# seceq/zkir

Measured on AMD Instinct MI355X. Metric: trace rows/sec (2^20-cycle fib: execution-trace fill + BabyBear NTT/LDE + Poseidon2 Merkle commitment), higher is better.
Workload: dtype u32 (Baby Bear, 31-bit modular) / u64 trace words

## Files before the change

include/zkir_amd.h:

```cpp
#ifndef ZKIR_AMD_H
#define ZKIR_AMD_H

#include <stddef.h>
#include <stdint.h>

#ifdef __cplusplus
extern "C" {
#endif

enum {
  ZKIR_OK = 0,
  ZKIR_ERR_MISALIGNED = 1,
  ZKIR_ERR_INVALID_MEMORY = 2,
  ZKIR_ERR_DIV_ZERO = 3,
  ZKIR_ERR_INVALID_SYSCALL = 4,
  ZKIR_ERR_DECODE = 5,
  ZKIR_ERR_OTHER = 6,
  ZKIR_ERR_BAD_PROGRAM = 7,
  ZKIR_ERR_DEVICE = 8,
  ZKIR_ERR_ARGUMENT = 9
};

enum { ZKIR_HALT_EBREAK = 0, ZKIR_HALT_EXIT = 1, ZKIR_HALT_CYCLE_LIMIT = 2 };

// ... 170 lines not shown
void zkir_stark_ctx_free(zkir_stark_ctx* ctx);
uint32_t zkir_main_trace_width(void);
uint32_t zkir_main_trace_width_for(uint32_t deferred);
uint32_t zkir_padded_log_n(uint64_t n_real);
int zkir_main_trace_launch(const zkir_trace_columns* trace, uint64_t n_real, uint32_t deferred, uint32_t* out, void* hip_stream);
typedef struct zkir_io_args { const uint64_t* inputs; uint64_t n_inputs; uint64_t writes_before, reads_before; } zkir_io_args;
int zkir_main_trace_io_launch(const zkir_trace_columns* trace, uint64_t n_real, const zkir_io_args* io, uint32_t* scratch, uint32_t* out, void* hip_stream);
int zkir_main_trace_io_host(const zkir_trace_columns* trace, uint64_t n_real, const zkir_io_args* io, uint32_t* out);
int zkir_main_trace_mem_launch(const zkir_trace_columns* trace, uint64_t n_real, const zkir_io_args* io, const uint64_t* mem_old, const uint32_t* mem_told, uint32_t* scratch, uint32_t* out,
                               void* hip_stream);
int zkir_main_trace_mem_host(const zkir_trace_columns* trace, uint64_t n_real, const zkir_io_args* io, const uint64_t* mem_old, const uint32_t* mem_told, uint32_t* out);
int zkir_main_trace_wide_launch(const zkir_trace_columns* trace, uint64_t n_real, const zkir_io_args* io, const uint64_t* mem_old, const uint32_t* mem_told, uint64_t code_size,
                                uint32_t* scratch, uint32_t* out, void* hip_stream);
int zkir_main_trace_wide_host(const zkir_trace_columns* trace, uint64_t n_real, const zkir_io_args* io, const uint64_t* mem_old, const uint32_t* mem_told, uint64_t code_size, uint32_t* out);
int zkir_main_trace_host(const zkir_trace_columns* trace, uint64_t n_real, uint32_t deferred, uint32_t* out);
void zkir_air_eval_host(const uint32_t* loc, const uint32_t* nxt, const uint32_t* aloc, const uint32_t* anxt, const uint32_t* lk, uint32_t is_first, uint32_t is_last, uint32_t is_trans,
                        const uint32_t* first68, const uint32_t* last68, const uint32_t* alpha4, uint32_t mode ,
                        const uint32_t* cnt4 , uint32_t* out4);
int zkir_air_check_bounds(uint32_t deferred, char* why, size_t why_len);
int zkir_lde_launch(const zkir_stark_ctx* ctx, uint32_t* in, uint32_t width, uint32_t* out, void* hip_stream);
int zkir_merkle_commit_launch(const zkir_stark_ctx* ctx, const uint32_t* mat, uint32_t width, uint64_t n_leaves, uint32_t* tree, void* hip_stream);

int zkir_merkle_leaves_launch(const zkir_stark_ctx* ctx, const uint32_t* mat, uint32_t width, uint64_t n_leaves, uint32_t* digests, void* hip_stream);

int zkir_merkle_cap_launch(const zkir_stark_ctx* ctx, uint32_t* tree, uint64_t n_digests, void* hip_stream);

typedef struct zkir_public_inputs {
  uint64_t n_real;
  uint64_t entry_point;
  uint32_t deferred;
  uint32_t fri_params;
  uint32_t program_digest[4];
  uint32_t io_digest[4];
  const uint8_t* program_blob;
  uint64_t program_blob_len;
  const uint64_t* inputs;
  uint64_t n_inputs;
  const uint64_t* outputs;
  uint64_t n_outputs;
  uint32_t halt_kind;
  uint32_t reserved2;
  uint64_t halt_code;
  uint64_t writes_before, reads_before;
  const uint64_t* mem_old;
  const uint32_t* mem_told;
  const uint64_t* cell_addr;
// ... 44 lines not shown
  uint32_t num_queries;
  uint32_t pow_bits;
} zkir_prover_params;
int zkir_public_inputs_set_params(zkir_public_inputs* pub, const zkir_prover_params* params);

int zkir_prove(const zkir_stark_ctx* ctx, const zkir_trace_columns* trace, const zkir_public_inputs* pub, uint32_t** proof_out, uint64_t* proof_words,
               float* stage_ms, void* hip_stream);
void zkir_proof_free(uint32_t* proof);
int zkir_prove_result(const zkir_result* result, const zkir_prover_params* params, uint8_t** proof, size_t* proof_len);
void zkir_proof_bytes_free(uint8_t* proof);
uint32_t zkir_proof_num_queries(void);
uint32_t zkir_proof_version(void);
uint32_t zkir_proof_version_of_mode(uint32_t mode);
int zkir_verify(const uint32_t* proof, uint64_t proof_words, const zkir_public_inputs* expect);
int zkir_verify_segment(const uint32_t* proof, uint64_t proof_words, const zkir_public_inputs* expect, uint32_t first_state[68], uint32_t last_state[68]);
int zkir_verify_chain(const uint32_t* const* proofs, const uint64_t* proof_words, uint32_t n_segments, const zkir_public_inputs* expect);
int zkir_verify_io(const uint32_t* proof, uint64_t words, const zkir_public_inputs* expect, const uint64_t* inputs, size_t n_inputs, const uint64_t* outputs, size_t n_outputs,
                   int halt_kind, uint64_t halt_code);
int zkir_verify_chain_io(const uint32_t* const* proofs, const uint64_t* words, uint32_t n_segments, const zkir_public_inputs* expect, const uint64_t* inputs, size_t n_inputs,
                         const uint64_t* outputs, size_t n_outputs, int halt_kind, uint64_t halt_code);
uint32_t zkir_proof_state_words(void);
void zkir_poseidon2_permute(uint32_t state[12]);
void zkir_poseidon2_permute_scaled(uint32_t state[12], uint32_t rounds);


int zkir_exec(const uint8_t* program_blob, size_t blob_len, const uint64_t* inputs, size_t n_inputs,
              const zkir_vm_config* cfg, zkir_result** out);
int zkir_exec_window(const uint8_t* program_blob, size_t blob_len, const uint64_t* inputs, size_t n_inputs, const zkir_vm_config* cfg,
                     uint64_t row_begin, uint64_t row_end, zkir_result** out);
int zkir_exec_shard(const zkir_delta_log* log, uint64_t row_begin, uint64_t row_end, zkir_result** out);
void zkir_result_free(zkir_result* r);
const zkir_delta_log* zkir_result_delta_log(const zkir_result* r);
const zkir_trace_columns* zkir_result_trace(const zkir_result* r);
void zkir_result_stage_ms(const zkir_result* r, float out[4]);
int zkir_result_copy_column(const zkir_result* r, int field, int reg, void* dst);


typedef struct zkir_memory_witness {
  uint64_t n_ops;
  uint64_t n_rows;
  zkir_memop_columns row_order;
  const uint64_t* row_offsets;
  zkir_memop_columns sorted;
} zkir_memory_witness;
int zkir_result_memory_trace(zkir_result* r, zkir_memory_witness* out);

// ... 41 lines not shown
```

zkir_amd/csrc/babybear.h:

```cpp
#pragma once
#include <cstdint>

#if defined(__HIPCC__)
#define BB_HD __host__ __device__ __forceinline__
#else
#define BB_HD inline
#endif

namespace bb {

constexpr uint32_t P = 0x78000001u;
constexpr uint32_t NEG_PINV = 0x77FFFFFFu;
constexpr uint32_t R1 = 0x0FFFFFFEu;
constexpr uint32_t R2 = 0x45DDDDE3u;
constexpr uint32_t GEN = 31u;
constexpr uint32_t ROOT27 = 0x1A427A41u;
constexpr uint32_t W_EXT = 11u;

BB_HD uint32_t add(uint32_t a, uint32_t b) { const uint32_t s = a + b, d = s - P; return d < s ? d : s; }
BB_HD uint32_t sub(uint32_t a, uint32_t b) { const uint32_t d = a - b, e = d + P; return e < d ? e : d; }
BB_HD uint32_t neg(uint32_t a) { return a ? P - a : 0u; }
BB_HD uint32_t dbl(uint32_t a) { return add(a, a); }
BB_HD uint32_t mont_mul(uint32_t a, uint32_t b) {
  const uint64_t t = (uint64_t)a * b;
// ... 138 lines not shown
#endif
}
BB_HD int32_t wredc(int64_t acc) {
#if defined(__HIP_DEVICE_COMPILE__)
  const int32_t m = (int32_t)((uint32_t)acc * NEG_PINV);
  return (int32_t)((uint64_t)wmadk<(int32_t)P>(acc, m) >> 32);
#else
  return smont_reduce_wide(acc);
#endif
}
BB_HD int32_t centre(uint32_t w) { const uint32_t u = w + (uint32_t)W_HALF, d = u - P; return (int32_t)((d < u ? d : u) - (uint32_t)W_HALF); }
BB_HD uint32_t wcanon(int32_t x) { const uint32_t u = (uint32_t)x, s = u + P; return s < u ? s : u; }
BB_HD int32_t mont_mul_centred(uint32_t a, uint32_t b) {
#if defined(__HIP_DEVICE_COMPILE__)
  uint64_t t, u;
  asm("v_mad_u64_u32 %0, vcc, %1, %2, %3" : "=v"(t) : "v"(a), "v"(b), "s"((uint64_t)(uint32_t)W_HALF << 32) : "vcc");
  const uint32_t m = (uint32_t)t * NEG_PINV;
  asm("v_mad_u64_u32 %0, vcc, %1, %2, %3" : "=v"(u) : "v"(m), "s"(P), "v"(t) : "vcc");
  return (int32_t)(reduce_2p((uint32_t)(u >> 32)) - (uint32_t)W_HALF);
#else
  return (int32_t)(reduce_2p(mont_mul_add_lazy(a, b, (uint64_t)(uint32_t)W_HALF << 32)) - (uint32_t)W_HALF);
#endif
}
BB_HD void dit2w(int32_t& a, int32_t& b, int32_t w, int32_t nw) {
  const int64_t A = wmulk<W_ONE>(a);
  const int32_t b0 = b;
  a = wredc(wmad(A, b0, w)); b = wredc(wmad(A, b0, nw));
}
BB_HD void dit4w(int32_t& x0, int32_t& x1, int32_t& x2, int32_t& x3, int32_t w1, int32_t n1, int32_t w2, int32_t n2, int32_t w2i, int32_t n2i) {
  const int64_t X0 = wmulk<W_ONE>(x0), X2 = wmulk<W_ONE>(x2);
  const int64_t y0 = wmad(X0, x1, w1), y1 = wmad(X0, x1, n1);
  const int32_t y2 = wredc(wmad(X2, x3, w1)), y3 = wredc(wmad(X2, x3, n1));
  x0 = wredc(wmad(y0, y2, w2)); x2 = wredc(wmad(y0, y2, n2));
  x1 = wredc(wmad(y1, y3, w2i)); x3 = wredc(wmad(y1, y3, n2i));
}
BB_HD void dit4w2(int32_t* a, int32_t* b, int32_t w1, int32_t n1, int32_t w2, int32_t n2, int32_t w2i, int32_t n2i) {
#if defined(__HIP_DEVICE_COMPILE__)
  int64_t ay0, ay1, at2, at3, by0, by1, bt2, bt3;
  asm("v_mad_i64_i32 %1, vcc, %8, %18, 0\n\tv_mad_i64_i32 %5, vcc, %12, %18, 0\n\t"
      "v_mad_i64_i32 %3, vcc, %10, %18, 0\n\tv_mad_i64_i32 %7, vcc, %14, %18, 0\n\t"
      "v_mad_i64_i32 %0, vcc, %9, %16, %1\n\tv_mad_i64_i32 %4, vcc, %13, %16, %5\n\t"
      "v_mad_i64_i32 %2, vcc, %11, %16, %3\n\tv_mad_i64_i32 %6, vcc, %15, %16, %7\n\t"
      "v_mad_i64_i32 %1, vcc, %9, %17, %1\n\tv_mad_i64_i32 %5, vcc, %13, %17, %5\n\t"
      "v_mad_i64_i32 %3, vcc, %11, %17, %3\n\tv_mad_i64_i32 %7, vcc, %15, %17, %7"
      : "=&v"(ay0), "=&v"(ay1), "=&v"(at2), "=&v"(at3), "=&v"(by0), "=&v"(by1), "=&v"(bt2), "=&v"(bt3)
      : "v"(a[0]), "v"(a[1]), "v"(a[2]), "v"(a[3]), "v"(b[0]), "v"(b[1]), "v"(b[2]), "v"(b[3]), "v"(w1), "v"(n1), "s"(W_ONE) : "vcc");
// ... 117 lines not shown
```

zkir_amd/csrc/ntt.hip:

```cpp
#include <hip/hip_runtime.h>

#include <atomic>
#include <cstdlib>
#include <mutex>
#include <type_traits>

#include "../../include/zkir_amd.h"
#include "../../include/zkir_amd_experimental.h"
#include "babybear.h"
#include "host.h"

namespace {

constexpr int NT = 256;
__device__ __forceinline__ uint32_t bitrev(uint32_t x, int bits) { return bits == 0 ? 0u : __brev(x) >> (32 - bits); }

template <int K, int N, class F>
__device__ __forceinline__ void static_for(F&& f) {
  if constexpr (K < N) { f(std::integral_constant<int, K>{}); static_for<K + 1, N>(f); }
}

using u32x4 = uint32_t __attribute__((ext_vector_type(4)));
__device__ __forceinline__ u32x4 ld4(const uint4* p) { return *reinterpret_cast<const u32x4*>(p); }
__device__ __forceinline__ void st4(uint4* p, u32x4 v) { *reinterpret_cast<u32x4*>(p) = v; }
// ... 336 lines not shown
    uint32_t v[2];
    int cnt = 0;
    for (uint32_t e = threadIdx.x; e < n; e += NT) { const uint32_t k = bitrev(e, L); v[cnt++] = bb::mont_mul(bb::mont_mul(lds[e], g_lo[k & 1023]), g_hi[k >> 10]); }
    __syncthreads();
    cnt = 0;
    for (uint32_t e = threadIdx.x; e < n; e += NT) { lds[2 * e] = v[cnt]; lds[2 * e + 1] = v[cnt]; cnt++; }
    __syncthreads();
    for (int s = 1; s <= L; s++) {
      const uint32_t half = 1u << s;
      for (uint32_t q = threadIdx.x; q < n; q += NT) {
        const uint32_t r_lo = q & (half - 1), r_hi = q >> s;
        const uint32_t ia = (r_hi << (s + 1)) | r_lo, ib = ia + half;
        const uint32_t a = lds[ia], t = bb::mont_mul(lds[ib], small_fwd[r_lo << (L - s)]);
        lds[ia] = bb::add(a, t); lds[ib] = bb::sub(a, t);
      }
      __syncthreads();
    }
    for (uint32_t e = threadIdx.x; e < 2 * n; e += NT) y[(uint64_t)e * 8 + c] = lds[e];
    __syncthreads();
  }
}

constexpr int MID_NT = 512;
__global__ __launch_bounds__(MID_NT) __attribute__((amdgpu_waves_per_eu(4, 4))) void lde_middle_r4_kernel(const uint4* __restrict__ in, uint4* __restrict__ out, uint32_t chunks_per_block, uint32_t total, int L,
                                                                const uint32_t* __restrict__ tw_inv, const uint32_t* __restrict__ small_inv, const uint32_t* __restrict__ small_fwd,
                                                                const uint32_t* __restrict__ g_lo, const uint32_t* __restrict__ g_hi, uint32_t j4_inv_m, uint32_t j4_fwd_m, int canon) {
  constexpr int Bm = 10;
  constexpr uint32_t APL = 1024;
  __shared__ uint4 A[2 * APL];
  __shared__ uint4 Bf[2048];
  const uint32_t n = 1u << L, t = threadIdx.x;
  uint32_t w = blockIdx.x;
  if (w >= total) return;
  uint32_t tw_i[5], tw_f[5];
#pragma unroll
  for (int r = 0; r < 5; r++) {
    const int lg = 8 - 2 * r;
    tw_i[r] = small_inv[bitrev((t & 255) >> lg, 2 * r) << lg];
    const int sft = 2 * r + 1;
    tw_f[r] = small_fwd[(t & ((1u << sft) - 1)) << (Bm - sft - 1)];
  }
  u32x4 pre[4];
  uint32_t cf_next[5];
  uint32_t glo[4], ghi[4];
  auto fetch = [&](uint32_t ww) {
    const uint4* x = in + ((uint64_t)(ww / chunks_per_block) * n + ((uint64_t)(ww % chunks_per_block) << Bm)) * 2;
#pragma unroll
    for (int k = 0; k < 4; k++) pre[k] = ld4(&x[t + k * MID_NT]);
    const uint32_t p0 = ((ww % chunks_per_block) << Bm) + 4 * (t & 255);
#pragma unroll
    for (int i = 0; i < 4; i++) { const uint32_t k = bitrev(p0 + i, L); glo[i] = g_lo[k & 1023]; ghi[i] = g_hi[k >> 10]; }
    const uint32_t ce = bitrev(ww % chunks_per_block, L - Bm);
#pragma unroll
    for (int r = 0; r < 5; r++) cf_next[r] = tw_inv[ce << (8 - 2 * r)];
  };
  fetch(w);
  for (;;) {
    const uint32_t base = (w % chunks_per_block) << Bm;
    uint4* y = out + (uint64_t)(w / chunks_per_block) * n * 4;
#pragma unroll
    for (int k = 0; k < 4; k++) { const uint32_t e = t + k * MID_NT; st4(&A[(e & 1) * APL + (e >> 1)], pre[k]); }
    uint32_t gs[4];
#pragma unroll
    for (int i = 0; i < 4; i++) gs[i] = bb::mont_mul(glo[i], ghi[i]);
// ... 11 lines not shown
        const int lg = 8 - 2 * r;
        const uint32_t h2 = 1u << lg, lo = q & (h2 - 1), hi = q >> lg;
        const uint32_t i0 = (hi << (lg + 2)) | lo;
        WTw c1, c2, c2i;
        ct_twiddles(tw_i[r], cf[r], false, j4_inv_m, c1, c2, c2i);
        uint4 x0 = a[i0], x1 = a[i0 + h2], x2 = a[i0 + 2 * h2], x3 = a[i0 + 3 * h2];
        ct4w4(x0, x1, x2, x3, c1, c2, c2i);
        if (r == 4) {
          x0 = scale4(x0, gs[0]); x1 = scale4(x1, gs[1]); x2 = scale4(x2, gs[2]); x3 = scale4(x3, gs[3]);
        }
        a[i0] = x0; a[i0 + h2] = x1; a[i0 + 2 * h2] = x2; a[i0 + 3 * h2] = x3;
        if (r >= 1 && r < 4) wave_sync_lds(); else __syncthreads();
      }
    }
#pragma unroll 1
    for (int h = 0; h < 2; h++) {
      const uint4* a = A + h * APL;
      uint4* F = h == 0 ? Bf : A;
#pragma unroll
      for (int r = 0; r < 5; r++) {
        const int s = 2 * r + 1;
        const uint32_t lo = t & ((1u << s) - 1), hi = t >> s;
        const uint32_t i0 = (hi << (s + 2)) | lo, d = 1u << s;
        const uint32_t w2 = tw_f[r];
        const WTw c2 = wtw(bb::centre(w2)), c1 = wtw(bb::mont_mul_centred(w2, w2)), c2i = wtw(bb::mont_mul_centred(w2, j4_fwd_m));
        uint4 x0, x1, x2, x3;
        if (r == 0) {
          x0 = a[i0 >> 1]; x1 = a[(i0 + d) >> 1]; x2 = a[(i0 + 2 * d) >> 1]; x3 = a[(i0 + 3 * d) >> 1];
          __syncthreads();
        } else { x0 = F[i0]; x1 = F[i0 + d]; x2 = F[i0 + 2 * d]; x3 = F[i0 + 3 * d]; }
        dit4w4(x0, x1, x2, x3, c1, c2, c2i);
        F[i0] = x0; F[i0 + d] = x1; F[i0 + 2 * d] = x2; F[i0 + 3 * d] = x3;
        if (r < 2) wave_sync_lds(); else __syncthreads();
      }
    }
#pragma unroll
    for (int k = 0; k < 4; k++) {
      const uint32_t e = t + k * MID_NT;
      uint4 v0 = Bf[e], v1 = A[e];
      if (canon) { v0 = canon4(v0); v1 = canon4(v1); }
      y[((uint64_t)2 * base + e) * 2] = v0; y[((uint64_t)2 * base + e) * 2 + 1] = v1;
    }
    __syncthreads();
    if (wn >= total) break;
    w = wn;
  }
}

// ... 75 lines not shown
```

zkir_amd/csrc/poseidon2.h:

```cpp
#pragma once
#include "babybear.h"

#ifndef P2_RF_UNROLL
#define P2_RF_UNROLL 1
#endif
namespace p2 {

constexpr int T = 12, RF = 8, RP = 22, RATE = 8, DIGEST = 4;

struct Consts {
  uint32_t ext[RF][T];
  uint32_t in[RP];
  uint32_t diag[T];
  uint32_t pre[RF][T];
  uint32_t ext0_s[T];
  uint64_t pre_b[RF][T];
  uint32_t in_scale;
  uint32_t out_scale;
  uint32_t carry;
  int32_t in0_neg;
  int32_t pr_c[RP];
  uint64_t pr_a[RP];
  uint64_t pr_k[T];
};

inline uint64_t splitmix64(uint64_t& s) {
  uint64_t z = (s += 0x9E3779B97F4A7C15ull);
// ... 227 lines not shown
  }
  int_round_a(x, t, w, c, RP - 1);
  s[0] = (uint32_t)x;
#pragma unroll
  for (int i = 1; i < T; i++) s[i] = (uint32_t)bb::smont_reduce_wide((int64_t)((uint64_t)w[i] + c.pr_k[i]));
}
BB_HD void permute_scaled(uint32_t* s, const Consts& c) {
  ext_linear_scaled<true>(s, c.ext0_s);
#pragma unroll P2_RF_UNROLL
  for (int r = 0; r < RF / 2; r++) {
#pragma unroll
    for (int i = 0; i < T; i++) s[i] = sbox_biased(s[i], c.pre_b[r][i]);
    ext_linear_scaled<false>(s, nullptr);
  }
  int_rounds_scaled(s, c);
#pragma unroll P2_RF_UNROLL
  for (int r = RF / 2; r < RF; r++) {
#pragma unroll
    for (int i = 0; i < T; i++) s[i] = sbox_biased(s[i], c.pre_b[r][i]);
    ext_linear_scaled<false>(s, nullptr);
  }
}

#if defined(__HIPCC__)
template <int CTRL>
__device__ __forceinline__ uint32_t quad_perm(uint32_t v) { return (uint32_t)__builtin_amdgcn_mov_dpp((int)v, CTRL, 0xF, 0xF, true); }
template <int CTRL>
__device__ __forceinline__ uint64_t quad_perm64(uint64_t v) { return ((uint64_t)quad_perm<CTRL>((uint32_t)(v >> 32)) << 32) | quad_perm<CTRL>((uint32_t)v); }

template <bool ADD_RC>
__device__ __forceinline__ void ext_linear_quad_scaled(uint32_t* s, const uint32_t* m4row, const uint32_t* rc) {
  uint64_t y[3];
#pragma unroll
  for (int b = 0; b < 3; b++) {
    const uint32_t v0 = quad_perm<0x00>(s[b]), v1 = quad_perm<0x55>(s[b]), v2 = quad_perm<0xAA>(s[b]), v3 = quad_perm<0xFF>(s[b]);
    y[b] = (uint64_t)v0 * m4row[0] + (uint64_t)v1 * m4row[1] + (uint64_t)v2 * m4row[2] + (uint64_t)v3 * m4row[3];
  }
  const uint64_t sum = y[0] + y[1] + y[2];
#pragma unroll
  for (int b = 0; b < 3; b++) {
    uint64_t v = y[b] + sum;
    if (ADD_RC) v += rc[b];
    s[b] = bb::mont_reduce_wide(v);
  }
}
__device__ __forceinline__ void int_round_quad(int32_t& x, int64_t* w, uint64_t mask0, const int* k, const Consts& c, int r) {
// ... 106 lines not shown
```

zkir_amd/csrc/stark.hip:

```cpp
#include <hip/hip_runtime.h>

#include <array>
#include <atomic>
#include <chrono>
#include <cstdio>
#include <cstdlib>
#include <cstddef>
#include <memory>
#include <mutex>
#include <vector>

#include "../../include/zkir_amd.h"
#include "../../include/zkir_amd_experimental.h"
#include "air.h"
#include "babybear.h"
#include "host.h"
#include "hashcall.h"
#include "poseidon2.h"
#include "verify_stages.h"

namespace {

constexpr int NT = 256;

// ... 420 lines not shown
  uint32_t d[8], pre[8];
  uint32_t run = bb::R1;
#pragma unroll
  for (int k = 0; k < 8; k++) {
    const uint32_t j = j0 + k;
    const uint32_t wj = j < N ? tw_fwd[j] : bb::neg(tw_fwd[j - N]);
    d[k] = bb::sub(bb::mont_mul(wj, bb::to_mont(bb::GEN)), bb::R1);
    pre[k] = run; run = bb::mont_mul(run, d[k]);
  }
  uint32_t inv = bb::R1, b = run, e = bb::P - 2;
  while (e) { if (e & 1) inv = bb::mont_mul(inv, b); b = bb::mont_mul(b, b); e >>= 1; }
#pragma unroll
  for (int k = 7; k >= 0; k--) { inv_xm1[j0 + k] = bb::mont_mul(inv, pre[k]); inv = bb::mont_mul(inv, d[k]); }
}


__global__ __launch_bounds__(NT) void leaf_hash_kernel(const p2::Consts* __restrict__ cp, const uint32_t* __restrict__ mat, uint32_t width, uint64_t n, uint32_t in_scale, uint32_t* __restrict__ digests) {
  const uint64_t j = (uint64_t)blockIdx.x * NT + threadIdx.x;
  if (j >= n) return;
  uint32_t s[p2::T];
#pragma unroll
  for (int i = 0; i < p2::T; i++) s[i] = 0;
  const uint4* m4 = reinterpret_cast<const uint4*>(mat);
  const uint32_t carry = cp->carry, out_scale = cp->out_scale;
  for (uint32_t off = 0; off < width; off += p2::RATE) {
    const uint4 lo = m4[((uint64_t)(off >> 3) * n + j) * 2], hi = m4[((uint64_t)(off >> 3) * n + j) * 2 + 1];
    const uint32_t v[8] = {lo.x, lo.y, lo.z, lo.w, hi.x, hi.y, hi.z, hi.w};
#pragma unroll
    for (int i = 0; i < p2::RATE; i++) s[i] = off + i < width ? bb::mont_mul_lazy(v[i], in_scale) : bb::mont_mul_lazy(s[i], carry);
#pragma unroll
    for (int i = p2::RATE; i < p2::T; i++) s[i] = bb::mont_mul_lazy(s[i], carry);
    p2::permute_scaled(s, *cp);
  }
  if (width == 0) p2::permute_scaled(s, *cp);
  uint4 d = make_uint4(bb::mont_mul(s[0], out_scale), bb::mont_mul(s[1], out_scale), bb::mont_mul(s[2], out_scale), bb::mont_mul(s[3], out_scale));
  reinterpret_cast<uint4*>(digests)[j] = d;
}

__global__ __launch_bounds__(NT) void leaf_absorb_kernel(const p2::Consts* __restrict__ cp, const uint32_t* __restrict__ mat, uint32_t width, uint32_t b0, uint32_t b1, uint64_t n, uint32_t in_scale,
                                                         uint4* __restrict__ state, int first, int last, uint32_t* __restrict__ digests) {
  const uint64_t j = (uint64_t)blockIdx.x * NT + threadIdx.x;
  if (j >= n) return;
  uint32_t s[p2::T];
  if (first) {
#pragma unroll
    for (int i = 0; i < p2::T; i++) s[i] = 0;
  } else {
    const uint4 a = state[j], b = state[n + j], c = state[2 * n + j];
    s[0] = a.x; s[1] = a.y; s[2] = a.z; s[3] = a.w; s[4] = b.x; s[5] = b.y; s[6] = b.z; s[7] = b.w; s[8] = c.x; s[9] = c.y; s[10] = c.z; s[11] = c.w;
  }
  const uint4* m4 = reinterpret_cast<const uint4*>(mat);
  const uint32_t carry = cp->carry, out_scale = cp->out_scale;
  for (uint32_t blk = b0; blk < b1; blk++) {
    const uint32_t off = blk * 8;
    const uint4 lo = m4[((uint64_t)blk * n + j) * 2], hi = m4[((uint64_t)blk * n + j) * 2 + 1];
    const uint32_t v[8] = {lo.x, lo.y, lo.z, lo.w, hi.x, hi.y, hi.z, hi.w};
#pragma unroll
    for (int i = 0; i < p2::RATE; i++) s[i] = off + i < width ? bb::mont_mul_lazy(v[i], in_scale) : bb::mont_mul_lazy(s[i], carry);
#pragma unroll
    for (int i = p2::RATE; i < p2::T; i++) s[i] = bb::mont_mul_lazy(s[i], carry);
    p2::permute_scaled(s, *cp);
  }
  if (last) {
    reinterpret_cast<uint4*>(digests)[j] = make_uint4(bb::mont_mul(s[0], out_scale), bb::mont_mul(s[1], out_scale), bb::mont_mul(s[2], out_scale), bb::mont_mul(s[3], out_scale));
  } else {
    state[j] = make_uint4(s[0], s[1], s[2], s[3]); state[n + j] = make_uint4(s[4], s[5], s[6], s[7]); state[2 * n + j] = make_uint4(s[8], s[9], s[10], s[11]);
  }
}

__global__ __launch_bounds__(NT) void compress_kernel(const p2::Consts* __restrict__ cp, const uint32_t* __restrict__ in, uint64_t n_out, uint32_t* __restrict__ out) {
  const uint64_t i = (uint64_t)blockIdx.x * NT + threadIdx.x;
  if (i >= n_out) return;
  const uint4 l = reinterpret_cast<const uint4*>(in)[2 * i], r = reinterpret_cast<const uint4*>(in)[2 * i + 1];
  const uint32_t k = cp->in_scale, ko = cp->out_scale;
  uint32_t s[p2::T] = {bb::mont_mul_lazy(l.x, k), bb::mont_mul_lazy(l.y, k), bb::mont_mul_lazy(l.z, k), bb::mont_mul_lazy(l.w, k), bb::mont_mul_lazy(r.x, k), bb::mont_mul_lazy(r.y, k),
                       bb::mont_mul_lazy(r.z, k), bb::mont_mul_lazy(r.w, k), 0, 0, 0, 0};
  p2::permute_scaled(s, *cp);
  reinterpret_cast<uint4*>(out)[i] = make_uint4(bb::mont_mul(s[0], ko), bb::mont_mul(s[1], ko), bb::mont_mul(s[2], ko), bb::mont_mul(s[3], ko));
}

constexpr uint32_t SUBTREE = 1024, NT_SUB = 1024;
__global__ __launch_bounds__(NT_SUB) void subtree_kernel(const p2::Consts* __restrict__ cp, uint32_t* cur, uint64_t m, uint32_t per_wg, uint32_t* counter) {
  __shared__ uint4 buf[SUBTREE];
  __shared__ uint32_t last_one;
  const uint32_t t = threadIdx.x;
  uint64_t pos0 = (uint64_t)blockIdx.x * per_wg;
  for (uint32_t e = t; e < per_wg; e += NT_SUB) {
    const uint4 v = reinterpret_cast<const uint4*>(cur)[pos0 + e];
    buf[e] = make_uint4(bb::to_mont(v.x), bb::to_mont(v.y), bb::to_mont(v.z), bb::to_mont(v.w));
  }
  __syncthreads();
 levels:
  for (uint32_t cnt = per_wg; cnt > 1; cnt >>= 1) {
    cur += 4 * m; m >>= 1; pos0 >>= 1;
    const uint32_t n_perm = cnt / 2;
    if (n_perm > NT_SUB / 16) {
      const bool active = t < n_perm;
      uint32_t s[p2::T];
      if (active) {
        const uint4 l = buf[2 * t], r = buf[2 * t + 1];
        const uint32_t k_in = bb::from_mont(cp->in_scale);
        s[0] = bb::mont_mul_lazy(l.x, k_in); s[1] = bb::mont_mul_lazy(l.y, k_in); s[2] = bb::mont_mul_lazy(l.z, k_in); s[3] = bb::mont_mul_lazy(l.w, k_in);
        s[4] = bb::mont_mul_lazy(r.x, k_in); s[5] = bb::mont_mul_lazy(r.y, k_in); s[6] = bb::mont_mul_lazy(r.z, k_in); s[7] = bb::mont_mul_lazy(r.w, k_in);
        s[8] = s[9] = s[10] = s[11] = 0;
      }
      __syncthreads();
      if (active) {
        p2::permute_scaled(s, *cp);
        const uint32_t ko = cp->out_scale, ko_m = bb::to_mont(ko);
        buf[t] = make_uint4(bb::mont_mul(s[0], ko_m), bb::mont_mul(s[1], ko_m), bb::mont_mul(s[2], ko_m), bb::mont_mul(s[3], ko_m));
        reinterpret_cast<uint4*>(cur)[pos0 + t] = make_uint4(bb::mont_mul(s[0], ko), bb::mont_mul(s[1], ko), bb::mont_mul(s[2], ko), bb::mont_mul(s[3], ko));
      }
    } else {
      const uint32_t pi = t >> 4, l = t & 15;
      const bool active = pi < n_perm;
      const uint32_t* words = reinterpret_cast<const uint32_t*>(buf);
      uint32_t s = 0;
      if (active && l < 8) s = bb::mont_mul_lazy(words[8 * pi + l], bb::from_mont(cp->in_scale));
      __syncthreads();
      if (active) {
        s = p2::permute_row16_scaled(s, (int)l, *cp);
        if (l < 4) {
          const uint32_t ko = cp->out_scale;
          reinterpret_cast<uint32_t*>(buf)[4 * pi + l] = bb::mont_mul(s, bb::to_mont(ko));
          cur[4 * (pos0 + pi) + l] = bb::mont_mul(s, ko);
        }
      }
    }
    __syncthreads();
  }
#if defined(__HIP_DEVICE_COMPILE__) && !defined(__gfx950__)
// ... 96 lines not shown

extern "C" {

uint32_t zkir_main_trace_width(void) { return air::committed_width(false); }
uint32_t zkir_main_trace_width_for(uint32_t deferred) { return air::committed_width((int)deferred); }

void zkir_poseidon2_permute(uint32_t state[12]) {
  static const p2::Consts consts = [] { p2::Consts c; p2::generate(c); return c; }();
  uint32_t s[p2::T];
  for (int i = 0; i < p2::T; i++) s[i] = bb::to_mont(state[i] % bb::P);
  p2::permute(s, consts);
  for (int i = 0; i < p2::T; i++) state[i] = bb::from_mont(s[i]);
}

void zkir_poseidon2_permute_scaled(uint32_t state[12], uint32_t rounds) {
  static const p2::Consts consts = [] { p2::Consts c; p2::generate(c); return c; }();
  uint32_t s[p2::T];
  for (int i = 0; i < p2::T; i++) s[i] = bb::mont_mul_lazy(state[i] % bb::P, consts.in_scale);
  for (uint32_t r = 0; r < rounds; r++) {
    if (r) for (int i = 0; i < p2::T; i++) s[i] = bb::mont_mul_lazy(s[i], consts.carry);
    p2::permute_scaled(s, consts);
  }
  for (int i = 0; i < p2::T; i++) state[i] = rounds ? bb::mont_mul(s[i], consts.out_scale) : state[i] % bb::P;
}

namespace { typedef uint32_t u32x4 __attribute__((ext_vector_type(4)));
__global__ __launch_bounds__(NT) void copy16_kernel(const u32x4* __restrict__ src, u32x4* __restrict__ dst, uint64_t n) {
  const uint64_t stride = (uint64_t)gridDim.x * NT;
  uint64_t i = (uint64_t)blockIdx.x * NT + threadIdx.x;
  for (; i + 3 * stride < n; i += 4 * stride) {
    const u32x4 a = __builtin_nontemporal_load(src + i), b = __builtin_nontemporal_load(src + i + stride), c = __builtin_nontemporal_load(src + i + 2 * stride), d = __builtin_nontemporal_load(src + i + 3 * stride);
    __builtin_nontemporal_store(a, dst + i); __builtin_nontemporal_store(b, dst + i + stride); __builtin_nontemporal_store(c, dst + i + 2 * stride); __builtin_nontemporal_store(d, dst + i + 3 * stride);
  }
  for (; i < n; i += stride) dst[i] = src[i];
} }
double zkir_hbm_copy_peak_gbs(uint64_t bytes, void* stream) {
  hipStream_t s = (hipStream_t)stream;
  const uint64_t n = (bytes >> 14) << 10;
  if (!n) return 0.0;
  u32x4 *a = nullptr, *b = nullptr;
  if (hipMalloc((void**)&a, n * 16) != hipSuccess) return 0.0;
  if (hipMalloc((void**)&b, n * 16) != hipSuccess) { (void)hipFree(a); return 0.0; }
  (void)hipMemsetAsync(a, 1, n * 16, s);
  hipEvent_t e0, e1;
  (void)hipEventCreate(&e0); (void)hipEventCreate(&e1);
  double best = 0.0;
// ... 208 lines not shown
    const uint32_t b0 = g * group, b1 = std::min(nb, b0 + group);
    zkir::lde_run(t, in + (uint64_t)b0 * N * 8, b1 - b0, out + (uint64_t)b0 * N2 * 8, s);
    (void)hipEventRecord(c->ov_group_ev[g], s); (void)hipStreamWaitEvent(c->ov_stream, c->ov_group_ev[g], 0);
    hipLaunchKernelGGL(leaf_absorb_kernel, dim3(grid_for(N2)), dim3(NT), 0, c->ov_stream, c->d_p2, out, width, b0, b1, N2, c->consts.in_scale, c->d_ov_state, g == 0 ? 1 : 0, g + 1 == n_groups ? 1 : 0, tree);
  }
  (void)hipEventRecord(c->ov_ev[1], c->ov_stream); (void)hipStreamWaitEvent(s, c->ov_ev[1], 0);
  launch_tree_levels(c->d_p2, tree, N2, c->sync, s);
  return check_launch("commit_overlapped");
}

int zkir_lde_launch(const zkir_stark_ctx* c, uint32_t* in, uint32_t width, uint32_t* out, void* stream) { return lde_launch(c, in, width, out, false, (hipStream_t)stream); }

int zkir_merkle_commit_launch(const zkir_stark_ctx* c, const uint32_t* mat, uint32_t width, uint64_t n_leaves, uint32_t* tree, void* stream) {
  hipStream_t s = (hipStream_t)stream;
  if (!c || n_leaves == 0 || (n_leaves & (n_leaves - 1))) { zkir::set_last_error({ZKIR_ERR_ARGUMENT, "merkle: null context, or n_leaves not a power of two"}); return ZKIR_ERR_ARGUMENT; }
  return merkle_commit(c, mat, width, n_leaves, tree, false, s);
}

int zkir_merkle_leaves_launch(const zkir_stark_ctx* c, const uint32_t* mat, uint32_t width, uint64_t n_leaves, uint32_t* digests, void* stream) {
  if (!c || !mat || !digests || n_leaves == 0) { zkir::set_last_error({ZKIR_ERR_ARGUMENT, "merkle leaves: null argument or no leaves"}); return ZKIR_ERR_ARGUMENT; }
  hipLaunchKernelGGL(leaf_hash_kernel, dim3(grid_for(n_leaves)), dim3(NT), 0, (hipStream_t)stream, c->d_p2, mat, width, n_leaves, c->consts.in_scale, digests);
  return check_launch("merkle_leaves");
}

int zkir_merkle_cap_launch(const zkir_stark_ctx* c, uint32_t* tree, uint64_t n_digests, void* stream) {
  if (!c || n_digests == 0 || (n_digests & (n_digests - 1))) { zkir::set_last_error({ZKIR_ERR_ARGUMENT, "merkle cap: null context, or n_digests not a power of two"}); return ZKIR_ERR_ARGUMENT; }
  launch_tree_levels(c->d_p2, tree, n_digests, c->sync, (hipStream_t)stream);
  return check_launch("merkle_cap");
}

}

#include "stark_prove.inl"
```

zkir_amd/runtime.py:

```python
from __future__ import annotations

import ctypes as C
import os
from dataclasses import dataclass
from typing import List, Optional, Sequence, Tuple

import numpy as np

from .spec import Program

_HERE = os.path.dirname(os.path.abspath(__file__))
_SO = os.environ.get("ZKIR_AMD_LIB") or os.path.join(_HERE, "libzkir_amd.so")

(ZKIR_OK, ERR_MISALIGNED, ERR_INVALID_MEMORY, ERR_DIV_ZERO, ERR_INVALID_SYSCALL, ERR_DECODE, ERR_OTHER, ERR_BAD_PROGRAM,
 ERR_DEVICE, ERR_ARGUMENT) = range(10)
HALT_EBREAK, HALT_EXIT, HALT_CYCLE_LIMIT = 0, 1, 2

REG_EVENT_DTYPE = np.dtype([("value", "<u8"), ("payload", "<u8"), ("max_bits", "<u4"), ("vis", "<u4"), ("reg", "u1"),
                            ("state", "u1"), ("tag", "u1"), ("pad", "u1", (5,))])
MEM_EVENT_DTYPE = np.dtype([("address", "<u8"), ("value", "<u8"), ("row", "<u4"), ("is_write", "u1"), ("width", "u1"), ("pad", "<u2")])
RC_EVENT_DTYPE = np.dtype([("value", "<u8"), ("pc", "<u8")])
NORM_EVENT_DTYPE = np.dtype([("cycle", "<u8"), ("pc", "<u8"), ("raw_value", "<u8"), ("reg", "u1"), ("state", "u1"), ("opcode", "u1"),
                             ("pad", "u1", (5,))])
SHA_BLOCK_DTYPE = np.dtype([("message_block", "<u4", (16,)), ("timestamp", "<u8")])
# ... 320 lines not shown
    L.zkir_hash_call_cells_host.restype = U64
    L.zkir_hash_call_cells_host.argtypes = [U64, U64, U64, U32, U64, C.POINTER(U64)]
    L.zkir_memcheck_witness_device_mode.restype = C.c_int
    L.zkir_memcheck_witness_device_mode.argtypes = [C.POINTER(TraceColumnsC), U64, C.c_char_p, C.c_size_t, U32, V, U64, V, V, V, V, V, U64, C.POINTER(U64), V, U64, C.POINTER(U64), V]
    if hasattr(L, "zkir_tape_table_side_launch"):
        L.zkir_tape_table_side_launch.restype = C.c_int; L.zkir_tape_table_side_launch.argtypes = [V, U64, V, V, U64, V, V, V, V, V, V]
        L.zkir_tape_table_side_host.restype = C.c_int; L.zkir_tape_table_side_host.argtypes = [V, U64, V, V, U64, V, V, V, V, V]
        L.zkir_hash_tape_check_launch.restype = C.c_int; L.zkir_hash_tape_check_launch.argtypes = [V, U64, U64, U64, C.POINTER(C.c_int), V]
        L.zkir_hash_tape_check_host.restype = C.c_int; L.zkir_hash_tape_check_host.argtypes = [V, U64, U64, U64, C.POINTER(C.c_int)]
    if hasattr(L, "zkir_verify_device"):
        L.zkir_hash_tape_new_bytes_launch.restype = C.c_int; L.zkir_hash_tape_new_bytes_launch.argtypes = [V, U64, V, V]
        L.zkir_hash_tape_new_bytes_host.restype = C.c_int; L.zkir_hash_tape_new_bytes_host.argtypes = [V, U64, V]
        L.zkir_verify_device.restype = C.c_int; L.zkir_verify_device.argtypes = [V, U64, C.POINTER(PublicInputsC), V]
        L.zkir_verify_last_stages.restype = C.c_int; L.zkir_verify_last_stages.argtypes = [V, C.POINTER(C.c_uint32)]
    L.zkir_prove_result.restype = C.c_int
    L.zkir_prove_result.argtypes = [V, C.POINTER(ProverParamsC), C.POINTER(C.POINTER(C.c_uint8)), C.POINTER(C.c_size_t)]
    L.zkir_proof_bytes_free.restype = None
    L.zkir_proof_bytes_free.argtypes = [C.POINTER(C.c_uint8)]
    L.zkir_proof_free.restype = None
    L.zkir_proof_free.argtypes = [C.POINTER(C.c_uint32)]
    L.zkir_proof_num_queries.restype = U32
    L.zkir_poseidon2_permute.restype = None; L.zkir_poseidon2_permute.argtypes = [C.c_void_p]
    L.zkir_poseidon2_permute_scaled.restype = None; L.zkir_poseidon2_permute_scaled.argtypes = [C.c_void_p, C.c_uint32]
    L.zkir_exec.restype = C.c_int
    L.zkir_exec.argtypes = [C.c_char_p, C.c_size_t, C.POINTER(C.c_uint64), C.c_size_t, C.POINTER(VmConfigC), C.POINTER(C.c_void_p)]
    L.zkir_result_free.argtypes = [C.c_void_p]
    L.zkir_result_free.restype = None
    L.zkir_result_delta_log.restype = C.c_void_p
    L.zkir_result_delta_log.argtypes = [C.c_void_p]
    L.zkir_result_trace.restype = C.POINTER(TraceColumnsC)
    L.zkir_result_trace.argtypes = [C.c_void_p]
    L.zkir_result_stage_ms.restype = None
    L.zkir_result_stage_ms.argtypes = [C.c_void_p, C.POINTER(C.c_float)]
    L.zkir_result_copy_column.restype = C.c_int
    L.zkir_result_copy_column.argtypes = [C.c_void_p, C.c_int, C.c_int, C.c_void_p]
    for name, st in [("memory_trace", MemoryWitnessC), ("range_check_witnesses", RangeCheckWitnessC),
                     ("normalization_witnesses", NormalizationWitnessC), ("sha256_witnesses", Sha256WitnessC)]:
        f = getattr(L, "zkir_result_" + name)
        f.restype = C.c_int
        f.argtypes = [C.c_void_p, C.POINTER(st)]
    L.zkir_host_to_device.restype = C.c_int
    L.zkir_host_to_device.argtypes = [C.c_void_p, C.c_void_p, C.c_size_t, C.c_void_p]
    L.zkir_device_to_host.restype = C.c_int
    L.zkir_device_to_host.argtypes = [C.c_void_p, C.c_void_p, C.c_size_t]
    _lib = L
    return L
# ... 443 lines not shown
```

Baseline: 193.1 million.

## Skip unused Poseidon2 output words and cache forward LDE twiddles in LDS

```diff
diff --git a/include/zkir_amd.h b/include/zkir_amd.h
--- a/include/zkir_amd.h
+++ b/include/zkir_amd.h
@@ -216,6 +216,7 @@
 int zkir_merkle_commit_launch(const zkir_stark_ctx* ctx, const uint32_t* mat, uint32_t width, uint64_t n_leaves, uint32_t* tree, void* hip_stream);
 
 int zkir_merkle_leaves_launch(const zkir_stark_ctx* ctx, const uint32_t* mat, uint32_t width, uint64_t n_leaves, uint32_t* digests, void* hip_stream);
+int zkir_merkle_leaves_mont_launch(const zkir_stark_ctx* ctx, const uint32_t* mat, uint32_t width, uint64_t n_leaves, uint32_t* digests, void* hip_stream);
 
 int zkir_merkle_cap_launch(const zkir_stark_ctx* ctx, uint32_t* tree, uint64_t n_digests, void* hip_stream);
 
@@ -306,6 +307,7 @@
 uint32_t zkir_proof_state_words(void);
 void zkir_poseidon2_permute(uint32_t state[12]);
 void zkir_poseidon2_permute_scaled(uint32_t state[12], uint32_t rounds);
+void zkir_poseidon2_sponge_scaled(const uint32_t* words, uint32_t n, uint32_t out4[4]);
 
 
 int zkir_exec(const uint8_t* program_blob, size_t blob_len, const uint64_t* inputs, size_t n_inputs,
diff --git a/zkir_amd/csrc/babybear.h b/zkir_amd/csrc/babybear.h
--- a/zkir_amd/csrc/babybear.h
+++ b/zkir_amd/csrc/babybear.h
@@ -184,6 +184,9 @@
   return (int32_t)(reduce_2p(mont_mul_add_lazy(a, b, (uint64_t)(uint32_t)W_HALF << 32)) - (uint32_t)W_HALF);
 #endif
 }
+struct FwdTw { int32_t c2, c1, c2i; };
+BB_HD FwdTw fwd_twiddles(uint32_t w2, uint32_t j4_m) { return FwdTw{centre(w2), mont_mul_centred(w2, w2), mont_mul_centred(w2, j4_m)}; }
+constexpr uint32_t fwd_tw_offset(int r) { return ((2u << (2 * r)) - 2u) / 3u; }
 BB_HD void dit2w(int32_t& a, int32_t& b, int32_t w, int32_t nw) {
   const int64_t A = wmulk<W_ONE>(a);
   const int32_t b0 = b;
diff --git a/zkir_amd/csrc/ntt.hip b/zkir_amd/csrc/ntt.hip
--- a/zkir_amd/csrc/ntt.hip
+++ b/zkir_amd/csrc/ntt.hip
@@ -382,6 +382,7 @@
 }
 
 constexpr int MID_NT = 512;
+constexpr uint32_t MID_TWF = bb::fwd_tw_offset(5);
 __global__ __launch_bounds__(MID_NT) __attribute__((amdgpu_waves_per_eu(4, 4))) void lde_middle_r4_kernel(const uint4* __restrict__ in, uint4* __restrict__ out, uint32_t chunks_per_block, uint32_t total, int L,
                                                                 const uint32_t* __restrict__ tw_inv, const uint32_t* __restrict__ small_inv, const uint32_t* __restrict__ small_fwd,
                                                                 const uint32_t* __restrict__ g_lo, const uint32_t* __restrict__ g_hi, uint32_t j4_inv_m, uint32_t j4_fwd_m, int canon) {
@@ -389,17 +390,22 @@
   constexpr uint32_t APL = 1024;
   __shared__ uint4 A[2 * APL];
   __shared__ uint4 Bf[2048];
+  __shared__ uint4 TWF[MID_TWF];
   const uint32_t n = 1u << L, t = threadIdx.x;
   uint32_t w = blockIdx.x;
   if (w >= total) return;
-  uint32_t tw_i[5], tw_f[5];
+  uint32_t tw_i[5];
 #pragma unroll
   for (int r = 0; r < 5; r++) {
     const int lg = 8 - 2 * r;
     tw_i[r] = small_inv[bitrev((t & 255) >> lg, 2 * r) << lg];
     const int sft = 2 * r + 1;
-    tw_f[r] = small_fwd[(t & ((1u << sft) - 1)) << (Bm - sft - 1)];
-  }
+    if (t < (1u << sft)) {
+      const bb::FwdTw e = bb::fwd_twiddles(small_fwd[t << (Bm - sft - 1)], j4_fwd_m);
+      TWF[bb::fwd_tw_offset(r) + t] = make_uint4((uint32_t)e.c2, (uint32_t)e.c1, (uint32_t)e.c2i, (uint32_t)-e.c2);
+    }
+  }
+  __syncthreads();
   u32x4 pre[4];
   uint32_t cf_next[5];
   uint32_t glo[4], ghi[4];
@@ -457,8 +463,8 @@
         const int s = 2 * r + 1;
         const uint32_t lo = t & ((1u << s) - 1), hi = t >> s;
         const uint32_t i0 = (hi << (s + 2)) | lo, d = 1u << s;
-        const uint32_t w2 = tw_f[r];
-        const WTw c2 = wtw(bb::centre(w2)), c1 = wtw(bb::mont_mul_centred(w2, w2)), c2i = wtw(bb::mont_mul_centred(w2, j4_fwd_m));
+        const uint4 tw = TWF[bb::fwd_tw_offset(r) + lo];
+        const WTw c2 = WTw{(int32_t)tw.x, (int32_t)tw.w}, c1 = wtw((int32_t)tw.y), c2i = wtw((int32_t)tw.z);
         uint4 x0, x1, x2, x3;
         if (r == 0) {
           x0 = a[i0 >> 1]; x1 = a[(i0 + d) >> 1]; x2 = a[(i0 + 2 * d) >> 1]; x3 = a[(i0 + 3 * d) >> 1];
diff --git a/zkir_amd/csrc/poseidon2.h b/zkir_amd/csrc/poseidon2.h
--- a/zkir_amd/csrc/poseidon2.h
+++ b/zkir_amd/csrc/poseidon2.h
@@ -3,6 +3,11 @@
 
 #ifndef P2_RF_UNROLL
 #define P2_RF_UNROLL 1
+#endif
+#if defined(__HIP_DEVICE_COMPILE__)
+#define P2_SCHED_FENCE() __builtin_amdgcn_sched_barrier(0)
+#else
+#define P2_SCHED_FENCE() ((void)0)
 #endif
 namespace p2 {
 
@@ -276,6 +281,71 @@
   }
 }
 
+template <int KEEP_FROM, int KEEP_TO>
+BB_HD void ext_linear_scaled_keep(uint32_t* s) {
+  static_assert(0 <= KEEP_FROM && KEEP_FROM < KEEP_TO && KEEP_TO <= T, "a non-empty range of state words");
+  uint64_t y[T];
+  m4_wide(s[0], s[1], s[2], s[3], y); m4_wide(s[4], s[5], s[6], s[7], y + 4); m4_wide(s[8], s[9], s[10], s[11], y + 8);
+  uint64_t sum[4];
+#pragma unroll
+  for (int j = 0; j < 4; j++) sum[j] = y[j] + y[4 + j] + y[8 + j];
+#pragma unroll
+  for (int k = KEEP_FROM; k < KEEP_TO; k++) s[k] = bb::mont_reduce_wide(y[k] + sum[k & 3]);
+}
+template <int KEEP_FROM, int KEEP_TO>
+BB_HD void permute_scaled_keep(uint32_t* s, const Consts& c) {
+  ext_linear_scaled<true>(s, c.ext0_s);
+#pragma unroll P2_RF_UNROLL
+  for (int r = 0; r < RF / 2; r++) {
+#pragma unroll
+    for (int i = 0; i < T; i++) s[i] = sbox_biased(s[i], c.pre_b[r][i]);
+    ext_linear_scaled<false>(s, nullptr);
+  }
+  int_rounds_scaled(s, c);
+#pragma unroll P2_RF_UNROLL
+  for (int r = RF / 2; r < RF - 1; r++) {
+#pragma unroll
+    for (int i = 0; i < T; i++) s[i] = sbox_biased(s[i], c.pre_b[r][i]);
+    ext_linear_scaled<false>(s, nullptr);
+  }
+#pragma unroll
+  for (int i = 0; i < T; i++) s[i] = sbox_biased(s[i], c.pre_b[RF - 1][i]);
+  P2_SCHED_FENCE();
+  ext_linear_scaled_keep<KEEP_FROM, KEEP_TO>(s);
+}
+template <class Load>
+BB_HD void sponge_scaled(uint32_t* s, uint32_t width, uint32_t in_scale, const Consts& c, Load&& load) {
+  const uint32_t carry = c.carry;
+  const uint32_t n_blocks = (width + RATE - 1) / RATE, n_full = width / RATE;
+  uint32_t v[RATE];
+  uint32_t b = 0;
+  for (; b + 1 < n_full; b++) {
+    load(b, v);
+#pragma unroll
+    for (int i = 0; i < RATE; i++) s[i] = bb::mont_mul_lazy(v[i], in_scale);
+#pragma unroll
+    for (int i = RATE; i < T; i++) s[i] = bb::mont_mul_lazy(s[i], carry);
+    permute_scaled_keep<RATE, T>(s, c);
+  }
+  if (b + 1 < n_blocks) {
+    load(b, v);
+#pragma unroll
+    for (int i = 0; i < RATE; i++) s[i] = bb::mont_mul_lazy(v[i], in_scale);
+#pragma unroll
+    for (int i = RATE; i < T; i++) s[i] = bb::mont_mul_lazy(s[i], carry);
+    permute_scaled(s, c);
+    b++;
+  }
+  if (b < n_blocks) {
+    load(b, v);
+#pragma unroll
+    for (int i = 0; i < RATE; i++) s[i] = b * RATE + i < width ? bb::mont_mul_lazy(v[i], in_scale) : bb::mont_mul_lazy(s[i], carry);
+#pragma unroll
+    for (int i = RATE; i < T; i++) s[i] = bb::mont_mul_lazy(s[i], carry);
+  }
+  permute_scaled_keep<0, DIGEST>(s, c);
+}
+
 #if defined(__HIPCC__)
 template <int CTRL>
 __device__ __forceinline__ uint32_t quad_perm(uint32_t v) { return (uint32_t)__builtin_amdgcn_mov_dpp((int)v, CTRL, 0xF, 0xF, true); }
diff --git a/zkir_amd/csrc/stark.hip b/zkir_amd/csrc/stark.hip
--- a/zkir_amd/csrc/stark.hip
+++ b/zkir_amd/csrc/stark.hip
@@ -466,17 +466,11 @@
 #pragma unroll
   for (int i = 0; i < p2::T; i++) s[i] = 0;
   const uint4* m4 = reinterpret_cast<const uint4*>(mat);
-  const uint32_t carry = cp->carry, out_scale = cp->out_scale;
-  for (uint32_t off = 0; off < width; off += p2::RATE) {
-    const uint4 lo = m4[((uint64_t)(off >> 3) * n + j) * 2], hi = m4[((uint64_t)(off >> 3) * n + j) * 2 + 1];
-    const uint32_t v[8] = {lo.x, lo.y, lo.z, lo.w, hi.x, hi.y, hi.z, hi.w};
-#pragma unroll
-    for (int i = 0; i < p2::RATE; i++) s[i] = off + i < width ? bb::mont_mul_lazy(v[i], in_scale) : bb::mont_mul_lazy(s[i], carry);
-#pragma unroll
-    for (int i = p2::RATE; i < p2::T; i++) s[i] = bb::mont_mul_lazy(s[i], carry);
-    p2::permute_scaled(s, *cp);
-  }
-  if (width == 0) p2::permute_scaled(s, *cp);
+  const uint32_t out_scale = cp->out_scale;
+  p2::sponge_scaled(s, width, in_scale, *cp, [&](uint32_t b, uint32_t* v) {
+    const uint4 lo = m4[((uint64_t)b * n + j) * 2], hi = m4[((uint64_t)b * n + j) * 2 + 1];
+    v[0] = lo.x; v[1] = lo.y; v[2] = lo.z; v[3] = lo.w; v[4] = hi.x; v[5] = hi.y; v[6] = hi.z; v[7] = hi.w;
+  });
   uint4 d = make_uint4(bb::mont_mul(s[0], out_scale), bb::mont_mul(s[1], out_scale), bb::mont_mul(s[2], out_scale), bb::mont_mul(s[3], out_scale));
   reinterpret_cast<uint4*>(digests)[j] = d;
 }
@@ -519,7 +513,7 @@
   const uint32_t k = cp->in_scale, ko = cp->out_scale;
   uint32_t s[p2::T] = {bb::mont_mul_lazy(l.x, k), bb::mont_mul_lazy(l.y, k), bb::mont_mul_lazy(l.z, k), bb::mont_mul_lazy(l.w, k), bb::mont_mul_lazy(r.x, k), bb::mont_mul_lazy(r.y, k),
                        bb::mont_mul_lazy(r.z, k), bb::mont_mul_lazy(r.w, k), 0, 0, 0, 0};
-  p2::permute_scaled(s, *cp);
+  p2::permute_scaled_keep<0, p2::DIGEST>(s, *cp);
   reinterpret_cast<uint4*>(out)[i] = make_uint4(bb::mont_mul(s[0], ko), bb::mont_mul(s[1], ko), bb::mont_mul(s[2], ko), bb::mont_mul(s[3], ko));
 }
 
@@ -550,7 +544,7 @@
       }
       __syncthreads();
       if (active) {
-        p2::permute_scaled(s, *cp);
+        p2::permute_scaled_keep<0, p2::DIGEST>(s, *cp);
         const uint32_t ko = cp->out_scale, ko_m = bb::to_mont(ko);
         buf[t] = make_uint4(bb::mont_mul(s[0], ko_m), bb::mont_mul(s[1], ko_m), bb::mont_mul(s[2], ko_m), bb::mont_mul(s[3], ko_m));
         reinterpret_cast<uint4*>(cur)[pos0 + t] = make_uint4(bb::mont_mul(s[0], ko), bb::mont_mul(s[1], ko), bb::mont_mul(s[2], ko), bb::mont_mul(s[3], ko));
@@ -693,6 +687,15 @@
     p2::permute_scaled(s, consts);
   }
   for (int i = 0; i < p2::T; i++) state[i] = rounds ? bb::mont_mul(s[i], consts.out_scale) : state[i] % bb::P;
+}
+
+void zkir_poseidon2_sponge_scaled(const uint32_t* words, uint32_t n, uint32_t out4[4]) {
+  static const p2::Consts consts = [] { p2::Consts c; p2::generate(c); return c; }();
+  uint32_t s[p2::T] = {};
+  p2::sponge_scaled(s, n, consts.in_scale, consts, [&](uint32_t b, uint32_t* v) {
+    for (uint32_t i = 0; i < (uint32_t)p2::RATE; i++) v[i] = b * p2::RATE + i < n ? words[b * p2::RATE + i] % bb::P : 0u;
+  });
+  for (int i = 0; i < p2::DIGEST; i++) out4[i] = bb::mont_mul(s[i], consts.out_scale);
 }
 
 namespace { typedef uint32_t u32x4 __attribute__((ext_vector_type(4)));
@@ -947,6 +950,11 @@
   hipLaunchKernelGGL(leaf_hash_kernel, dim3(grid_for(n_leaves)), dim3(NT), 0, (hipStream_t)stream, c->d_p2, mat, width, n_leaves, c->consts.in_scale, digests);
   return check_launch("merkle_leaves");
 }
+int zkir_merkle_leaves_mont_launch(const zkir_stark_ctx* c, const uint32_t* mat, uint32_t width, uint64_t n_leaves, uint32_t* digests, void* stream) {
+  if (!c || !mat || !digests || n_leaves == 0) { zkir::set_last_error({ZKIR_ERR_ARGUMENT, "merkle leaves: null argument or no leaves"}); return ZKIR_ERR_ARGUMENT; }
+  hipLaunchKernelGGL(leaf_hash_kernel, dim3(grid_for(n_leaves)), dim3(NT), 0, (hipStream_t)stream, c->d_p2, mat, width, n_leaves, bb::from_mont(c->consts.in_scale), digests);
+  return check_launch("merkle_leaves_mont");
+}
 
 int zkir_merkle_cap_launch(const zkir_stark_ctx* c, uint32_t* tree, uint64_t n_digests, void* stream) {
   if (!c || n_digests == 0 || (n_digests & (n_digests - 1))) { zkir::set_last_error({ZKIR_ERR_ARGUMENT, "merkle cap: null context, or n_digests not a power of two"}); return ZKIR_ERR_ARGUMENT; }
diff --git a/zkir_amd/runtime.py b/zkir_amd/runtime.py
--- a/zkir_amd/runtime.py
+++ b/zkir_amd/runtime.py
@@ -366,6 +366,9 @@
     L.zkir_proof_num_queries.restype = U32
     L.zkir_poseidon2_permute.restype = None; L.zkir_poseidon2_permute.argtypes = [C.c_void_p]
     L.zkir_poseidon2_permute_scaled.restype = None; L.zkir_poseidon2_permute_scaled.argtypes = [C.c_void_p, C.c_uint32]
+    if hasattr(L, "zkir_poseidon2_sponge_scaled"):
+        L.zkir_merkle_leaves_mont_launch.restype = C.c_int; L.zkir_merkle_leaves_mont_launch.argtypes = [V, V, U32, U64, V, V]
+        L.zkir_poseidon2_sponge_scaled.restype = None; L.zkir_poseidon2_sponge_scaled.argtypes = [C.c_void_p, C.c_uint32, C.c_void_p]
     L.zkir_exec.restype = C.c_int
     L.zkir_exec.argtypes = [C.c_char_p, C.c_size_t, C.POINTER(C.c_uint64), C.c_size_t, C.POINTER(VmConfigC), C.POINTER(C.c_void_p)]
     L.zkir_result_free.argtypes = [C.c_void_p]
```

Measured after the change: 194.5 million, median of 6. Within noise of the previous version (+0.7%).
